# 20171130/Equivariant-NN-Zoo

Hardware: AMD Instinct MI355X
Metric: molecules/s forward+backward, QM9 config_energy batch (higher is better)
Workload: dtype f32

## Files before the change

### equivariant-nn-zoo_amd/csrc/e3k_node.hip

```cpp
#include "e3k_common.h"
#include "e3k_act.h"

namespace e3k {

__global__ __launch_bounds__(256) void act_fwd_kernel(const float* __restrict__ x, int64_t n, int act, float cst,
                                                       float* __restrict__ y) {
  for (int64_t i = (int64_t)blockIdx.x * 256 + threadIdx.x; i < n; i += (int64_t)gridDim.x * 256)
    y[i] = cst * act_f(act, x[i]);
}
__global__ __launch_bounds__(256) void act_bwd_kernel(const float* __restrict__ x, const float* __restrict__ gy,
                                                       int64_t n, int act, float cst, float* __restrict__ gx) {
  for (int64_t i = (int64_t)blockIdx.x * 256 + threadIdx.x; i < n; i += (int64_t)gridDim.x * 256)
    gx[i] = gy[i] * cst * act_df(act, x[i]);
}

__global__ __launch_bounds__(256) void act_bwd2_kernel(const float* __restrict__ x, const float* __restrict__ gy,
                                                        const float* __restrict__ gh, int64_t n, int act, float cst,
                                                        float* __restrict__ g_gy, float* __restrict__ g_x) {
  for (int64_t i = (int64_t)blockIdx.x * 256 + threadIdx.x; i < n; i += (int64_t)gridDim.x * 256) {
    const float xv = x[i], h = gh[i] * cst;
    if (g_gy) g_gy[i] = h * act_df(act, xv);
    if (g_x) g_x[i] = h * gy[i] * act_d2f(act, xv);
  }
}
// ... 246 lines not shown
        case 3: gate_bwd_gated<CF, 3>(s, xr, gr, gr2, gxr, u); break;
        case 5: gate_bwd_gated<CF, 5>(s, xr, gr, gr2, gxr, u); break;
        default: gate_bwd_gated<CF, 7>(s, xr, gr, gr2, gxr, u); break;
      }
    }
  }
}

template <int CF, int DIM>
__device__ __forceinline__ void gate_fwd_gated(const e3k_gate_seg& s, const float* __restrict__ xr, float* __restrict__ yr, int u) {
  float xv[DIM][4];
  const float4 xg4 = ld4(xr + s.gate_off + u);
#pragma unroll
  for (int m = 0; m < DIM; ++m) {
    const float4 a = ld4(xr + s.in_off + m * s.mul + u);
    xv[m][0] = a.x; xv[m][1] = a.y; xv[m][2] = a.z; xv[m][3] = a.w;
  }
  const float sc[4] = {s.cst * act_f(s.act, xg4.x), s.cst * act_f(s.act, xg4.y), s.cst * act_f(s.act, xg4.z),
                       s.cst * act_f(s.act, xg4.w)};
  if (CF) {
#pragma unroll
    for (int m = 0; m < DIM; ++m)
      st4(yr + s.out_off + m * s.mul + u, xv[m][0] * sc[0], xv[m][1] * sc[1], xv[m][2] * sc[2], xv[m][3] * sc[3]);
  } else {
    float v[4 * DIM];
#pragma unroll
    for (int j = 0; j < 4; ++j)
#pragma unroll
      for (int m = 0; m < DIM; ++m) v[j * DIM + m] = xv[m][j] * sc[j];
#pragma unroll
    for (int k = 0; k < DIM; ++k) st4(yr + s.out_off + u * DIM + 4 * k, v[4 * k], v[4 * k + 1], v[4 * k + 2], v[4 * k + 3]);
  }
}

template <int CF>
__global__ __launch_bounds__(256) void gate_fwd4_kernel(const float* __restrict__ x, int64_t rows, int in_dim, int out_dim,
                                                         GateArgs ga, int rb, float* __restrict__ y) {
  const e3k_gate_seg& s = ga.s[blockIdx.y];
  const int q = s.mul >> 2;
  const int64_t row0 = (int64_t)blockIdx.x * rb;
  for (int i = threadIdx.x; i < rb * q; i += 256) {
    const int rr = i / q, u = (i - rr * q) * 4;
    const int64_t r = row0 + rr;
    if (r >= rows) break;
    const float* xr = x + r * in_dim;
    float* yr = y + r * out_dim;
    if (s.kind == 0) {
      const float4 xc = ld4(xr + s.in_off + u);
      st4(yr + s.out_off + u, s.cst * act_f(s.act, xc.x), s.cst * act_f(s.act, xc.y), s.cst * act_f(s.act, xc.z),
          s.cst * act_f(s.act, xc.w));
    } else {
      switch (s.dim) {
        case 1: gate_fwd_gated<CF, 1>(s, xr, yr, u); break;
        case 3: gate_fwd_gated<CF, 3>(s, xr, yr, u); break;
        case 5: gate_fwd_gated<CF, 5>(s, xr, yr, u); break;
        default: gate_fwd_gated<CF, 7>(s, xr, yr, u); break;
      }
    }
  }
}

__global__ __launch_bounds__(256) void gate_bwd2_gy_kernel(const float* __restrict__ x, const float* __restrict__ gh,
                                                            int64_t rows, int in_dim, int out_dim, GateArgs ga,
                                                            float* __restrict__ g_gy) {
  const int c = blockIdx.x * 256 + threadIdx.x;
  if (c >= out_dim) return;
  for (int64_t r = blockIdx.y; r < rows; r += gridDim.y) {
    const int64_t i = r * out_dim + c;
    const float* xr = x + r * in_dim;
    const float* hr = gh + r * in_dim;
    float v = 0.f;
    for (int k = 0; k < ga.n; ++k) {
      const e3k_gate_seg& s = ga.s[k];
      const int rel = c - s.out_off;
      if (rel >= 0 && rel < s.mul * s.dim) {
        if (s.kind == 0) {
          v = hr[s.in_off + rel] * s.cst * act_df(s.act, xr[s.in_off + rel]);
        } else {
          int u, m;
          gate_out_um(s, rel, ga.out_cf, u, m);
          const float gt = xr[s.gate_off + u];
          const int xi = s.in_off + m * s.mul + u;
          v = hr[xi] * (s.cst * act_f(s.act, gt)) + hr[s.gate_off + u] * xr[xi] * (s.cst * act_df(s.act, gt));
        }
        break;
      }
    }
    g_gy[i] = v;
  }
}

__global__ __launch_bounds__(256) void gate_bwd2_x_kernel(const float* __restrict__ x, const float* __restrict__ gy,
                                                           const float* __restrict__ gh, int64_t rows, int in_dim,
                                                           int out_dim, GateArgs ga, float* __restrict__ g_x) {
  const int c = blockIdx.x * 256 + threadIdx.x;
  if (c >= in_dim) return;
  for (int64_t r = blockIdx.y; r < rows; r += gridDim.y) {
    const int64_t i = r * in_dim + c;
    const float* xr = x + r * in_dim;
    const float* hr = gh + r * in_dim;
    const float* gr = gy + r * out_dim;
    float v = 0.f;
    for (int k = 0; k < ga.n; ++k) {
      const e3k_gate_seg& s = ga.s[k];
      if (s.kind == 0) {
        const int rel = c - s.in_off;
        if (rel >= 0 && rel < s.mul) {
          v = hr[c] * gr[s.out_off + rel] * s.cst * act_d2f(s.act, xr[c]);
          break;
        }
      } else {
        const int relg = c - s.gate_off;
        if (relg >= 0 && relg < s.mul) {
          float dgh = 0.f, dgx = 0.f;
          for (int m = 0; m < s.dim; ++m) {
            const float g = gr[gate_out_idx(s, relg, m, ga.out_cf)];
            dgh = fmaf(g, hr[s.in_off + m * s.mul + relg], dgh);
            dgx = fmaf(g, xr[s.in_off + m * s.mul + relg], dgx);
          }
          v = s.cst * (dgh * act_df(s.act, xr[c]) + hr[c] * dgx * act_d2f(s.act, xr[c]));
          break;
        }
        const int rel = c - s.in_off;
        if (rel >= 0 && rel < s.mul * s.dim) {
          const int m = rel / s.mul, u = rel - m * s.mul;
          v = hr[s.gate_off + u] * gr[gate_out_idx(s, u, m, ga.out_cf)] * (s.cst * act_df(s.act, xr[s.gate_off + u]));
          break;
        }
      }
    }
    g_x[i] = v;
  }
}

constexpr int KW_MAXI = 16, KW_MAXV = 32, KW_MAXK = 1 << 22;
struct KwArgs {
  int n, K, V;
  int64_t ld_m, total;
  e3k_kw_instr ins[KW_MAXI];
};

__device__ __forceinline__ const float* kw_locate(const KwArgs& ka, int64_t c, const float* W, int& wout) {
  int j = 0;
  for (int i = 1; i < ka.n; ++i)
    if (c >= ka.ins[i].m_off) j = i;
  const e3k_kw_instr& in = ka.ins[j];
  const int local = (int)(c - in.m_off);
  const int u = local / in.w_out, w = local - u * in.w_out;
  wout = in.w_out;
  return W + in.w_off + (int64_t)u * ka.V * in.w_out + w;
}

constexpr int KW_KT = 64, KW_KT_WIDE = 512;
static inline unsigned kw_tiles(int n_keys, int64_t col_blocks) {
  const int kt = col_blocks >= 1024 ? KW_KT_WIDE : KW_KT;
  return (unsigned)((n_keys + kt - 1) / kt);
}
template <int MODE>
__device__ __forceinline__ void kw_body(const float* __restrict__ a, const float* __restrict__ W, const KwArgs& ka, const int K,
                                        float* __restrict__ M, float* __restrict__ Wout_, int accumulate) {
  const int tile = uniform((K + (int)gridDim.y - 1) / (int)gridDim.y);
  const int t0 = uniform((int)blockIdx.y * tile);
  const int kt = (K - t0 < tile) ? K - t0 : tile;
  if (kt <= 0) return;
  const int V = uniform(ka.V);
  const int64_t c = (int64_t)blockIdx.x * 256 + threadIdx.x;
  if (c >= ka.total) return;
  int wout;
  const float* base = kw_locate(ka, c, W, wout);
  if constexpr (MODE == 0) {
    float wv[KW_MAXV];
#pragma unroll
    for (int v = 0; v < KW_MAXV; ++v) wv[v] = v < V ? base[(int64_t)v * wout] : 0.f;
    for (int t = 0; t < kt; ++t) {
      const float* __restrict__ ar = a + (int64_t)(t0 + t) * V;
      float acc = 0.f;
#pragma unroll
      for (int v = 0; v < KW_MAXV; ++v)
        if (v < V) acc = fmaf(ar[v], wv[v], acc);
      M[(int64_t)(t0 + t) * ka.ld_m + c] = acc;
    }
  } else {
    float gv[KW_MAXV];
#pragma unroll
    for (int v = 0; v < KW_MAXV; ++v) gv[v] = 0.f;
    for (int t = 0; t < kt; ++t) {
      const float* __restrict__ ar = a + (int64_t)(t0 + t) * V;
      const float g = M[(int64_t)(t0 + t) * ka.ld_m + c];
#pragma unroll
      for (int v = 0; v < KW_MAXV; ++v)
        if (v < V) gv[v] = fmaf(ar[v], g, gv[v]);
    }
    float* dst = Wout_ + (base - W);
    if (gridDim.y == 1) {
#pragma unroll
      for (int v = 0; v < KW_MAXV; ++v)
        if (v < V) dst[(int64_t)v * wout] = accumulate ? dst[(int64_t)v * wout] + gv[v] : gv[v];
    } else {
#pragma unroll
      for (int v = 0; v < KW_MAXV; ++v)
        if (v < V) atomicAdd(dst + (int64_t)v * wout, gv[v]);
    }
  }
}

template <int MODE>
__global__ __launch_bounds__(256) void keyed_weights_kernel(const float* __restrict__ a, const float* __restrict__ W,
                                                             KwArgs ka, float* __restrict__ M, float* __restrict__ Wout_,
                                                             int accumulate) {
  kw_body<MODE>(a, W, ka, ka.K, M, Wout_, accumulate);
}

constexpr int KW_MAXL = 8;
struct KwMulti {
  int n, K;
  const KwArgs* ka[KW_MAXL];
  const float* W[KW_MAXL];
  float* M[KW_MAXL];
  float* gW[KW_MAXL];
  int acc[KW_MAXL];
  int64_t ws_off[KW_MAXL];
};
template <int MODE>
__global__ __launch_bounds__(256) void keyed_weights_multi_kernel(const float* __restrict__ a, KwMulti m) {
  const int z = blockIdx.z;
  if (MODE == 1 && !m.gW[z]) return;
  kw_body<MODE>(a, m.W[z], *m.ka[z], m.K, m.M[z], m.gW[z], m.acc[z]);
}

constexpr int KWA_COLS = 256, KWA_KT = 16, KWA_RANGE = 128;
constexpr int KWA_WLD = KWA_COLS + 4;
__device__ __forceinline__ void kw_bwd_a_body(const float* __restrict__ gM, const float* __restrict__ W, const KwArgs& ka_,
                                              const int K, float* __restrict__ ws, float (*gs)[KWA_COLS], float (*wsm)[KWA_WLD]) {
  struct { int K, V; int64_t ld_m, total; } ka{K, ka_.V, ka_.ld_m, ka_.total};
  const int t_id = threadIdx.x;
  const int64_t c = (int64_t)blockIdx.x * KWA_COLS + t_id;
  const bool ok = c < ka.total;
  {
    int wout = 1;
    const float* base = ok ? kw_locate(ka_, c, W, wout) : W;
    for (int v = 0; v < ka.V; ++v) wsm[v][t_id] = ok ? base[(int64_t)v * wout] : 0.f;
  }
  float* out = ws + (int64_t)blockIdx.x * ka.K * ka.V;
  const int t_begin = blockIdx.y * KWA_RANGE;
  const int t_end = (t_begin + KWA_RANGE < ka.K) ? t_begin + KWA_RANGE : ka.K;
  for (int t0 = t_begin; t0 < t_end; t0 += KWA_KT) {
    const int kt = (t_end - t0 < KWA_KT) ? t_end - t0 : KWA_KT;
    __syncthreads();
    for (int t = 0; t < kt; ++t) gs[t][t_id] = ok ? gM[(int64_t)(t0 + t) * ka.ld_m + c] : 0.f;
    __syncthreads();
    for (int o = t_id; o < kt * ka.V; o += 256) {
      const int t = o / ka.V, v = o - t * ka.V;
      const float4* g4 = reinterpret_cast<const float4*>(gs[t]);
      const float4* w4 = reinterpret_cast<const float4*>(wsm[v]);
      float acc = 0.f;
#pragma unroll 8
      for (int q = 0; q < KWA_COLS / 4; ++q) {
        const float4 g = g4[q], w = w4[q];
        acc = fmaf(g.x, w.x, acc);
        acc = fmaf(g.y, w.y, acc);
        acc = fmaf(g.z, w.z, acc);
        acc = fmaf(g.w, w.w, acc);
      }
      out[(t0 + t) * ka.V + v] = acc;
    }
  }
}

__global__ __launch_bounds__(256) void keyed_weights_bwd_a_kernel(const float* __restrict__ gM, const float* __restrict__ W,
                                                                   KwArgs ka, float* __restrict__ ws) {
  __shared__ __attribute__((aligned(16))) float gs[KWA_KT][KWA_COLS];
  __shared__ __attribute__((aligned(16))) float wsm[KW_MAXV][KWA_WLD];
  kw_bwd_a_body(gM, W, ka, ka.K, ws, gs, wsm);
}

__global__ __launch_bounds__(256) void keyed_weights_bwd_a_multi_kernel(KwMulti m, float* __restrict__ ws) {
  __shared__ __attribute__((aligned(16))) float gs[KWA_KT][KWA_COLS];
  __shared__ __attribute__((aligned(16))) float wsm[KW_MAXV][KWA_WLD];
  const int z = blockIdx.z;
  const KwArgs& ka = *m.ka[z];
  if ((int64_t)blockIdx.x * KWA_COLS >= ka.total) return;
  kw_bwd_a_body(m.M[z], m.W[z], ka, m.K, ws + m.ws_off[z] * m.K * ka.V, gs, wsm);
}

__global__ __launch_bounds__(256) void keyed_weights_bwd_a_reduce_kernel(const float* __restrict__ ws, int n_rows, int n,
                                                                          float* __restrict__ ga) {
  const int o = blockIdx.x * 4 + (threadIdx.x >> 6), lane = threadIdx.x & 63;
  if (o >= n) return;
  float acc = 0.f;
  for (int r = lane; r < n_rows; r += 64) acc += ws[(int64_t)r * n + o];
  acc = wave_sum(acc);
  if (lane == 0) ga[o] += acc;
}

__device__ __forceinline__ void normact_scale(int act, float eps2, int normalize, float n2, float& s, float& ds_over_n) {
  if (eps2 > 0.f) {
    const bool clamped = n2 < eps2;
    const float n = sqrtf(clamped ? eps2 : n2);
    const float a = act_f(act, n), da = act_df(act, n);
    if (normalize) {
      s = a / n;
      ds_over_n = clamped ? 0.f : (da * n - a) / (n * n * n);
    } else {
      s = a;
      ds_over_n = clamped ? 0.f : da / n;
    }
  } else {
    s = act_f(act, n2);
    ds_over_n = 2.0f * act_df(act, n2);
  }
}

__global__ __launch_bounds__(256) void normact_fwd_kernel(const float* __restrict__ x, int64_t rows, int row_dim,
                                                           BlockArgs ba, int act, float eps2, int normalize,
                                                           float* __restrict__ y) {
  const int64_t total = rows * row_dim;
  for (int64_t i = (int64_t)blockIdx.x * 256 + threadIdx.x; i < total; i += (int64_t)gridDim.x * 256) {
    const int64_t r = i / row_dim;
    const int c = (int)(i - r * row_dim);
    const float* xr = x + r * row_dim;
    float v = 0.f;
    for (int k = 0; k < ba.n; ++k) {
      const e3k_block& b = ba.b[k];
      const int rel = c - b.off;
      if (rel >= 0 && rel < b.mul * b.dim) {
        const int u = rel / b.dim, m = rel - u * b.dim;
        float n2 = 0.f;
        for (int q = 0; q < b.dim; ++q) {
          const float t = xr[b.off + q * b.mul + u];
          n2 = fmaf(t, t, n2);
        }
        float s, d;
        normact_scale(act, eps2, normalize, n2, s, d);
        v = s * xr[b.off + m * b.mul + u];
        break;
      }
    }
    y[i] = v;
  }
}

__device__ __forceinline__ void normact_scale2(int act, float eps2, int normalize, float n2, float& s, float& d, float& d2) {
  if (eps2 > 0.f) {
    const bool clamped = n2 < eps2;
    const float n = sqrtf(clamped ? eps2 : n2);
    const float a = act_f(act, n), a1 = act_df(act, n), a2 = act_d2f(act, n);
    float s1, s2;
    if (normalize) {
      s = a / n;
      s1 = (a1 * n - a) / (n * n);
      s2 = (a2 * n * n - 2.0f * a1 * n + 2.0f * a) / (n * n * n);
    } else {
      s = a;
      s1 = a1;
      s2 = a2;
    }
    d = clamped ? 0.f : s1 / n;
    d2 = clamped ? 0.f : (s2 * n - s1) / (n * n * n);
  } else {
    s = act_f(act, n2);
    d = 2.0f * act_df(act, n2);
    d2 = 4.0f * act_d2f(act, n2);
  }
}

__global__ __launch_bounds__(256) void normact_bwd2_kernel(const float* __restrict__ x, const float* __restrict__ gy,
                                                            const float* __restrict__ h, int64_t rows, int row_dim, BlockArgs ba,
                                                            int act, float eps2, int normalize, float* __restrict__ g_gy,
                                                            float* __restrict__ g_x) {
  const int64_t total = rows * row_dim;
  for (int64_t i = (int64_t)blockIdx.x * 256 + threadIdx.x; i < total; i += (int64_t)gridDim.x * 256) {
    const int64_t r = i / row_dim;
    const int c = (int)(i - r * row_dim);
    const float* xr = x + r * row_dim;
    const float* gr = gy + r * row_dim;
    const float* hr = h + r * row_dim;
    bool covered = false;
    for (int k = 0; k < ba.n; ++k) {
      const e3k_block& b = ba.b[k];
      const int rel = c - b.off;
      if (rel >= 0 && rel < b.mul * b.dim) {
        covered = true;
        const int m = rel / b.mul, u = rel - m * b.mul;
        float n2 = 0.f, gx_ = 0.f, hx = 0.f, hg = 0.f;
        for (int q = 0; q < b.dim; ++q) {
          const float t = xr[b.off + q * b.mul + u], g = gr[b.off + u * b.dim + q], hh = hr[b.off + q * b.mul + u];
          n2 = fmaf(t, t, n2);
          gx_ = fmaf(g, t, gx_);
          hx = fmaf(hh, t, hx);
          hg = fmaf(hh, g, hg);
        }
        float s, d, d2;
        normact_scale2(act, eps2, normalize, n2, s, d, d2);
        const float xm = xr[c], hm = hr[c], gm = gr[b.off + u * b.dim + m];
        if (g_gy) g_gy[r * row_dim + b.off + u * b.dim + m] = fmaf(s, hm, d * hx * xm);
        if (g_x) g_x[i] = d * xm * hg + d2 * xm * hx * gx_ + d * (hm * gx_ + hx * gm);
        break;
      }
    }
    if (!covered) {
      if (g_gy) g_gy[i] = 0.f;
      if (g_x) g_x[i] = 0.f;
    }
// ... 759 lines not shown
```

### equivariant-nn-zoo_amd/csrc/e3k_rtable.hip

```cpp
#include "e3k_common.h"
#include "e3k_rtable_bwd.h"

namespace e3k {


constexpr int RT_CHUNK = 1024;
__global__ __launch_bounds__(256) void rtable_bins_rank_kernel(const float* __restrict__ r, const int64_t* __restrict__ key, int64_t E,
                                                               float h_inv, int32_t K, int32_t KT, int32_t* __restrict__ bin,
                                                               float* __restrict__ coef, int32_t* __restrict__ lrank,
                                                               int32_t* __restrict__ chunk_hist, int32_t* __restrict__ bad) {
  extern __shared__ int32_t hist_all[];
  const int lane = threadIdx.x & 63, wv = threadIdx.x >> 6;
  int32_t* hist = hist_all + wv * (KT + 1);
  const int64_t chunk = blockIdx.x;
  for (int b = threadIdx.x; b < 4 * (KT + 1); b += 256) hist_all[b] = 0;
  __syncthreads();
  constexpr int PER_WAVE = RT_CHUNK / 4 / 64;
  const int64_t base = chunk * RT_CHUNK + (int64_t)wv * (RT_CHUNK / 4);
  int my_bin[PER_WAVE], my_rank[PER_WAVE];
#pragma unroll
  for (int it = 0; it < PER_WAVE; ++it) {
    const int64_t e = base + it * 64 + lane;
    const bool live = e < E;
    int i = 1;
    if (live) {
      const float raw = r[e] * h_inv;
      float x = raw < 0.f ? 0.f : (raw > (float)K ? (float)K : raw);
      i = (int)x;
      i = i < 1 ? 1 : (i > K - 2 ? K - 2 : i);
      const float t = x - (float)i;
      const float tm1 = t - 1.f, tm2 = t - 2.f, tp1 = t + 1.f;
      float4 c;
      c.x = -t * tm1 * tm2 * (1.f / 6.f);
      c.y = tp1 * tm1 * tm2 * 0.5f;
      c.z = -tp1 * t * tm2 * 0.5f;
      c.w = tp1 * t * tm1 * (1.f / 6.f);
      if (key) {
        const int64_t kk = key[e];
        const int nk = (KT + 1) / (K + 1);
        const bool in_range = kk >= 0 && kk < nk;
        i += in_range ? (int)kk * (K + 1) : 0;
        if (!in_range && bad) atomicOr(bad, 8);
      }
      bin[e] = i;
      *reinterpret_cast<float4*>(coef + 4 * e) = c;
    }
    unsigned long long todo = __ballot(live);
    int rank = 0;
    while (todo) {
      const int leader = __ffsll((long long)todo) - 1;
      const int b = __shfl(i, leader, 64);
      const unsigned long long same = __ballot(live && i == b) & todo;
      const int seen = hist[b];
      if (live && i == b) rank = seen + __popcll(same & ((1ull << lane) - 1ull));
      if (lane == leader) hist[b] = seen + __popcll(same);
      todo &= ~same;
    }
    my_bin[it] = live ? i : -1;
    my_rank[it] = rank;
  }
  __syncthreads();
#pragma unroll
  for (int it = 0; it < PER_WAVE; ++it) {
    if (my_bin[it] < 0) continue;
    int before = 0;
    for (int w = 0; w < wv; ++w) before += hist_all[w * (KT + 1) + my_bin[it]];
    lrank[base + it * 64 + lane] = my_rank[it] + before;
  }
  for (int b = threadIdx.x; b <= KT; b += 256)
    chunk_hist[chunk * (KT + 1) + b] = hist_all[b] + hist_all[(KT + 1) + b] + hist_all[2 * (KT + 1) + b] + hist_all[3 * (KT + 1) + b];
}

__global__ __launch_bounds__(1024) void rtable_bins_scan_kernel(int32_t* __restrict__ chunk_hist, int32_t n_chunks, int32_t K,
                                                                int32_t* __restrict__ ptr, int32_t* __restrict__ seg) {
  __shared__ int32_t wave_tot[2][16];
  __shared__ int32_t carry[2];
  const int t = threadIdx.x, lane = t & 63, w = t >> 6;
  if (t < 2) carry[t] = 0;
  __syncthreads();
  for (int base = 0; base <= K; base += 1024) {
    const int b = base + t;
    int32_t cnt = 0;
    if (b <= K) {
      for (int c = 0; c < n_chunks; ++c) {
        const int32_t v = chunk_hist[(int64_t)c * (K + 1) + b];
        chunk_hist[(int64_t)c * (K + 1) + b] = cnt;
        cnt += v;
      }
    }
    const int32_t sg = (cnt + RT_SEG - 1) / RT_SEG;
    int32_t x = cnt, y = sg;
#pragma unroll
    for (int off = 1; off < 64; off <<= 1) {
      const int32_t xx = __shfl_up(x, off, 64), yy = __shfl_up(y, off, 64);
      if (lane >= off) x += xx, y += yy;
    }
    if (lane == 63) wave_tot[0][w] = x, wave_tot[1][w] = y;
    __syncthreads();
    int32_t bx = carry[0], by = carry[1];
    for (int k = 0; k < w; ++k) bx += wave_tot[0][k], by += wave_tot[1][k];
    if (b <= K) {
      ptr[b] = bx + x - cnt;
      seg[b] = by + y - sg;
      if (b == K) ptr[K + 1] = bx + x, seg[K + 1] = by + y;
    }
    __syncthreads();
    if (t == 1023) carry[0] = bx + x, carry[1] = by + y;
    __syncthreads();
  }
}

__global__ __launch_bounds__(256) void rtable_bins_place_kernel(const int32_t* __restrict__ bin, const int32_t* __restrict__ lrank,
                                                                const int32_t* __restrict__ chunk_off, const int32_t* __restrict__ ptr,
                                                                int64_t E, int32_t K, int32_t* __restrict__ perm) {
  const int64_t e = (int64_t)blockIdx.x * 256 + threadIdx.x;
  if (e >= E) return;
  const int b = bin[e];
  perm[ptr[b] + chunk_off[(e / RT_CHUNK) * (K + 1) + b] + lrank[e]] = (int32_t)e;
}

__global__ __launch_bounds__(256) void rtable_interp_fwd_kernel(const float* __restrict__ T, const int32_t* __restrict__ perm,
                                                                const int32_t* __restrict__ bin, const float* __restrict__ coef,
                                                                int64_t E, int32_t W, float* __restrict__ w,
                                                                const float* __restrict__ T2, float* __restrict__ w2) {
  const int64_t p = (int64_t)blockIdx.x * 4 + (threadIdx.x >> 6);
  if (p >= E) return;
  const int lane = threadIdx.x & 63;
  const int e = uniform(perm[p]);
  const int i = uniform(bin[e]);
  const float* __restrict__ cp = coef + 4 * (int64_t)e;
  const float c0 = __uint_as_float(uniform((int)__float_as_uint(cp[0]))), c1 = __uint_as_float(uniform((int)__float_as_uint(cp[1])));
  const float c2 = __uint_as_float(uniform((int)__float_as_uint(cp[2]))), c3 = __uint_as_float(uniform((int)__float_as_uint(cp[3])));
  const float4* __restrict__ a = reinterpret_cast<const float4*>(T + (int64_t)(i - 1) * W);
  const float4* __restrict__ b = reinterpret_cast<const float4*>(T + (int64_t)i * W);
  const float4* __restrict__ c = reinterpret_cast<const float4*>(T + (int64_t)(i + 1) * W);
  const float4* __restrict__ d = reinterpret_cast<const float4*>(T + (int64_t)(i + 2) * W);
  float4* __restrict__ o = reinterpret_cast<float4*>(w + (int64_t)e * W);
  for (int q = lane; q < (W >> 2); q += 64) {
    const float4 va = a[q], vb = b[q], vc = c[q], vd = d[q];
    float4 v;
    v.x = fmaf(c3, vd.x, fmaf(c2, vc.x, fmaf(c1, vb.x, c0 * va.x)));
    v.y = fmaf(c3, vd.y, fmaf(c2, vc.y, fmaf(c1, vb.y, c0 * va.y)));
    v.z = fmaf(c3, vd.z, fmaf(c2, vc.z, fmaf(c1, vb.z, c0 * va.z)));
    v.w = fmaf(c3, vd.w, fmaf(c2, vc.w, fmaf(c1, vb.w, c0 * va.w)));
    nt_store4(o + q, v);
  }
  if (T2) {
    const int64_t d2 = T2 - T;
    float4* __restrict__ o2 = reinterpret_cast<float4*>(w2 + (int64_t)e * W);
    for (int q = lane; q < (W >> 2); q += 64) {
      const float4 va = reinterpret_cast<const float4*>(reinterpret_cast<const float*>(a) + d2)[q];
      const float4 vb = reinterpret_cast<const float4*>(reinterpret_cast<const float*>(b) + d2)[q];
      const float4 vc = reinterpret_cast<const float4*>(reinterpret_cast<const float*>(c) + d2)[q];
      const float4 vd = reinterpret_cast<const float4*>(reinterpret_cast<const float*>(d) + d2)[q];
      float4 v;
      v.x = fmaf(c3, vd.x, fmaf(c2, vc.x, fmaf(c1, vb.x, c0 * va.x)));
      v.y = fmaf(c3, vd.y, fmaf(c2, vc.y, fmaf(c1, vb.y, c0 * va.y)));
      v.z = fmaf(c3, vd.z, fmaf(c2, vc.z, fmaf(c1, vb.z, c0 * va.z)));
      v.w = fmaf(c3, vd.w, fmaf(c2, vc.w, fmaf(c1, vb.w, c0 * va.w)));
      nt_store4(o2 + q, v);
    }
  }
}

__global__ __launch_bounds__(256) void rtable_bwd_partial_kernel(const float* __restrict__ gw, const float* __restrict__ coef,
                                                                 const float* __restrict__ scale,
                                                                 const int32_t* __restrict__ ptr, const int32_t* __restrict__ seg,
                                                                 const int32_t* __restrict__ perm, int32_t K, int32_t W,
                                                                 int32_t n_chunks, int64_t n_seg_cap, float* __restrict__ P) {
  rtable_bwd_partial_body<8>(gw, coef, scale, ptr, seg, perm, K, W, n_chunks, n_seg_cap, P, (int64_t)blockIdx.x);
}

__global__ __launch_bounds__(256) void rtable_bwd_combine_kernel(const float* __restrict__ P, const int32_t* __restrict__ seg,
                                                                 int32_t K, int32_t W, int32_t accumulate, float* __restrict__ gT) {
  const int64_t q = (int64_t)blockIdx.x * 256 + threadIdx.x;
  const int w4 = W >> 2;
  if (q >= (int64_t)(K + 1) * w4) return;
  const int j = (int)(q / w4), col = (int)(q - (int64_t)j * w4) * 4;
  float4 acc = make_float4(0.f, 0.f, 0.f, 0.f);
  float4* out = reinterpret_cast<float4*>(gT + (int64_t)j * W + col);
  if (accumulate) acc = *out;
#pragma unroll
  for (int k = 0; k < 4; ++k) {
    const int b = j + 1 - k;
    if (b < 1 || b > K - 2) continue;
    const int s0 = seg[b], s1 = seg[b + 1];
    for (int s = s0; s < s1; ++s) {
      const float4 v = *reinterpret_cast<const float4*>(P + ((int64_t)s * 4 + k) * W + col);
      acc.x += v.x; acc.y += v.y; acc.z += v.z; acc.w += v.w;
    }
  }
  *out = acc;
}

typedef _Float16 f16x2 __attribute__((ext_vector_type(2)));
constexpr float PK_S2 = 1024.f, PK_S3 = 65536.f;

__global__ __launch_bounds__(256) void rtable_pack_kernel(const float* __restrict__ T, int32_t K, int32_t W, uint32_t* __restrict__ P) {
  const int64_t q = (int64_t)blockIdx.x * 256 + threadIdx.x;
  if (q >= (int64_t)(K + 1) * W) return;
  const int i = (int)(q / W), col = (int)(q - (int64_t)i * W);
  uint32_t* row = P + 3 * (int64_t)i * W;
  if (i < 1 || i > K - 2) {
    row[2 * col] = row[2 * col + 1] = row[2 * W + col] = 0u;
    return;
  }
  const double a = T[q - W], b = T[q], c = T[q + W], d = T[q + 2 * (int64_t)W];
  const double c1 = -a / 3.0 - b / 2.0 + c - d / 6.0, c2 = a / 2.0 - b + c / 2.0, c3 = -a / 6.0 + b / 2.0 - c / 2.0 + d / 6.0;
  const double e2 = c2 + 1.5 * c3;
  f16x2 h;
  h.x = (_Float16)(float)(e2 * (double)PK_S2);
  h.y = (_Float16)(float)(c3 * (double)PK_S3);
  const double r2 = e2 - (double)(float)h.x / (double)PK_S2, r3 = c3 - (double)(float)h.y / (double)PK_S3;
  const float d0 = (float)(b + c1 / 2.0 + c2 / 4.0 + c3 / 8.0 + r2 / 8.0), d1 = (float)(c1 + c2 + 0.75 * c3 + 3.0 * r3 / 16.0);
  row[2 * col] = __float_as_uint(d0);
  row[2 * col + 1] = __float_as_uint(d1);
  row[2 * W + col] = __builtin_bit_cast(uint32_t, h);
}

struct PackMulti {
  const float* T[16];
  uint32_t* P[16];
  int32_t W[16];
};
__global__ __launch_bounds__(256) void rtable_pack_multi_kernel(PackMulti a, int32_t K) {
  const int tb = blockIdx.y;
  const int32_t W = a.W[tb];
  const int64_t q = (int64_t)blockIdx.x * 256 + threadIdx.x;
  if (q >= (int64_t)(K + 1) * W) return;
  const float* __restrict__ T = a.T[tb];
  const int i = (int)(q / W), col = (int)(q - (int64_t)i * W);
  uint32_t* row = a.P[tb] + 3 * (int64_t)i * W;
  if (i < 1 || i > K - 2) {
    row[2 * col] = row[2 * col + 1] = row[2 * W + col] = 0u;
    return;
  }
  const double ta = T[q - W], b = T[q], c = T[q + W], d = T[q + 2 * (int64_t)W];
  const double c1 = -ta / 3.0 - b / 2.0 + c - d / 6.0, c2 = ta / 2.0 - b + c / 2.0, c3 = -ta / 6.0 + b / 2.0 - c / 2.0 + d / 6.0;
  const double e2 = c2 + 1.5 * c3;
  f16x2 h;
  h.x = (_Float16)(float)(e2 * (double)PK_S2);
  h.y = (_Float16)(float)(c3 * (double)PK_S3);
  const double r2 = e2 - (double)(float)h.x / (double)PK_S2, r3 = c3 - (double)(float)h.y / (double)PK_S3;
  const float d0 = (float)(b + c1 / 2.0 + c2 / 4.0 + c3 / 8.0 + r2 / 8.0), d1 = (float)(c1 + c2 + 0.75 * c3 + 3.0 * r3 / 16.0);
  row[2 * col] = __float_as_uint(d0);
  row[2 * col + 1] = __float_as_uint(d1);
  row[2 * W + col] = __builtin_bit_cast(uint32_t, h);
}

__device__ __forceinline__ float packed_eval(float s, float s2, float s3, float d0, float d1, uint32_t pk) {
  const f16x2 h = __builtin_bit_cast(f16x2, pk);
  return fmaf(s, fmaf(s2, fmaf(s3, (float)h.y, (float)h.x), d1), d0);
}

__global__ __launch_bounds__(256) void rtable_interp_packed_kernel(const uint32_t* __restrict__ P, const int32_t* __restrict__ perm,
                                                                   const int32_t* __restrict__ bin, const float* __restrict__ coef,
                                                                   int64_t E, int32_t W, float* __restrict__ w) {
  const int64_t p = (int64_t)blockIdx.x * 4 + (threadIdx.x >> 6);
  if (p >= E) return;
  const int lane = threadIdx.x & 63;
  const int e = uniform(perm[p]);
  const int i = uniform(bin[e]);
  const float* __restrict__ cp = coef + 4 * (int64_t)e;
  const float c0 = __uint_as_float(uniform((int)__float_as_uint(cp[0]))), c2 = __uint_as_float(uniform((int)__float_as_uint(cp[2])));
  const float c3 = __uint_as_float(uniform((int)__float_as_uint(cp[3])));
  const float s = fmaf(2.f, c3, c2 - c0) - 0.5f, s2 = s * (1.f / PK_S2), s3 = s * (PK_S2 / PK_S3);
  const uint32_t* __restrict__ row = P + 3 * (int64_t)i * W;
  float* __restrict__ o = w + (int64_t)e * W;
  for (int q = lane; q < W; q += 64) o[q] = packed_eval(s, s2, s3, __uint_as_float(row[2 * q]), __uint_as_float(row[2 * q + 1]), row[2 * W + q]);
}

struct GuardArgs {
  const float* T[16];
  float* state[16];
  float* scratch[16];
  int32_t W[16];
  int32_t rows;
  float floor_rel, c4, col_weight, pack_weight;
};

__device__ __forceinline__ void atomic_max_pos(float* p, float v) {
  atomicMax(reinterpret_cast<unsigned int*>(p), __float_as_uint(v));
}

constexpr int RT_GUARD_PARTS = 8;
__global__ __launch_bounds__(256) void rtable_guard_kernel(GuardArgs a) {
  __shared__ float s_col[4][64], s_d4[4][64];
  const int tb = blockIdx.y;
  const int W = a.W[tb];
  const int n_chunks = (W + 63) / 64;
  if ((int)blockIdx.x >= n_chunks) return;
  const float* __restrict__ T = a.T[tb];
  const int lane = threadIdx.x & 63, q = threadIdx.x >> 6;
  const int col = blockIdx.x * 64 + lane;
  const int rows = a.rows;
  const int n_d4 = rows - 4;
  const int per = (n_d4 + 4 * RT_GUARD_PARTS - 1) / (4 * RT_GUARD_PARTS);
  const int rq = blockIdx.z * 4 + q;
  const int lo = rq * per < n_d4 ? rq * per : n_d4, hi = (lo + per < n_d4) ? lo + per : n_d4;
  float cmax = 0.f, dmax = 0.f;
  bool bad = false;
  if (col < W && lo < hi) {
    float v0 = T[(int64_t)lo * W + col], v1 = T[(int64_t)(lo + 1) * W + col], v2 = T[(int64_t)(lo + 2) * W + col],
          v3 = T[(int64_t)(lo + 3) * W + col];
    cmax = fmaxf(fmaxf(fabsf(v0), fabsf(v1)), fmaxf(fabsf(v2), fabsf(v3)));
    bad = !(fabsf(v0) < INFINITY) || !(fabsf(v1) < INFINITY) || !(fabsf(v2) < INFINITY) || !(fabsf(v3) < INFINITY);
    for (int i = lo; i < hi; ++i) {
      const float v4 = T[(int64_t)(i + 4) * W + col];
      bad = bad || !(fabsf(v4) < INFINITY);
      cmax = fmaxf(cmax, fabsf(v4));
      const float d4 = (v4 + v0) - 4.f * (v3 + v1) + 6.f * v2;
      const float d2 = (v1 + v3) - 2.f * v2, d3 = (v3 - v0) - 3.f * (v2 - v1);
      dmax = fmaxf(dmax, a.c4 * fabsf(d4) + a.pack_weight * (1.f / 2048.f) * (fabsf(d2) * (1.f / 16.f) + fabsf(d3) * (1.f / 192.f)));
      v0 = v1; v1 = v2; v2 = v3; v3 = v4;
    }
  }
  s_col[q][lane] = bad ? INFINITY : cmax;
  s_d4[q][lane] = bad ? INFINITY : dmax;
  __syncthreads();
  if (q == 0 && col < W) {
    float* __restrict__ mine = a.scratch[tb] + (int64_t)blockIdx.z * 2 * W;
    mine[col] = fmaxf(fmaxf(s_col[0][lane], s_col[1][lane]), fmaxf(s_col[2][lane], s_col[3][lane]));
    mine[W + col] = fmaxf(fmaxf(s_d4[0][lane], s_d4[1][lane]), fmaxf(s_d4[2][lane], s_d4[3][lane]));
  }
}

__global__ __launch_bounds__(256) void rtable_guard_reduce_kernel(GuardArgs a) {
  __shared__ float s_red[4], s_red2[4];
  const int tb = blockIdx.x;
  const int W = a.W[tb];
  const float* __restrict__ scratch = a.scratch[tb];
  const int lane = threadIdx.x & 63, q = threadIdx.x >> 6;
  float g = 0.f;
  auto fold = [&](int c, float& cm, float& dm) {
    cm = 0.f, dm = 0.f;
#pragma unroll
    for (int z = 0; z < RT_GUARD_PARTS; ++z) {
      cm = fmaxf(cm, scratch[(int64_t)z * 2 * W + c]);
      dm = fmaxf(dm, scratch[(int64_t)z * 2 * W + W + c]);
    }
  };
  for (int c = threadIdx.x; c < W; c += 256) {
// ... 186 lines not shown
```

Measured before the change: 94990.

## Batch loads for memory-level parallelism across keyed-weight and rtable kernels

The keyed-weights forward and backward bodies now handle keys in blocks of 4/2/1 and load activation chunks up front. The backward preloads old weight values and gradient rows. The bwd-a kernel prefetches the next gradient tile into registers while the current tile is computed. The rtable rank kernel swaps the serial leader loop for a fixed 64-step readlane/ballot match, and the scan and combine kernels batch their loads. All of this aims to hide memory latency by keeping more loads in flight, at the cost of more registers and possibly lower occupancy.

```diff
diff --git a/equivariant-nn-zoo_amd/csrc/e3k_node.hip b/equivariant-nn-zoo_amd/csrc/e3k_node.hip
--- a/equivariant-nn-zoo_amd/csrc/e3k_node.hip
+++ b/equivariant-nn-zoo_amd/csrc/e3k_node.hip
@@ -422,9 +422,48 @@
 }
 
 constexpr int KW_KT = 64, KW_KT_WIDE = 512;
+constexpr int KW_SB = 4, KW_KB = 8, KW_VC = 4;
 static inline unsigned kw_tiles(int n_keys, int64_t col_blocks) {
   const int kt = col_blocks >= 1024 ? KW_KT_WIDE : KW_KT;
   return (unsigned)((n_keys + kt - 1) / kt);
+}
+template <int NB, class F>
+__device__ __forceinline__ void kw_chunks(const float* __restrict__ ab, const int V, F&& f) {
+#pragma unroll
+  for (int v0 = 0; v0 < KW_MAXV; v0 += KW_VC) {
+    if (v0 + KW_VC <= V) {
+      float x[NB][KW_VC];
+#pragma unroll
+      for (int i = 0; i < NB; ++i)
+#pragma unroll
+        for (int q = 0; q < KW_VC; ++q) x[i][q] = ab[i * V + v0 + q];
+#pragma unroll
+      for (int i = 0; i < NB; ++i)
+#pragma unroll
+        for (int q = 0; q < KW_VC; ++q) f(i, v0 + q, x[i][q]);
+    } else if (v0 < V) {
+#pragma unroll
+      for (int q = 0; q < KW_VC - 1; ++q)
+        if (v0 + q < V) {
+#pragma unroll
+          for (int i = 0; i < NB; ++i) f(i, v0 + q, ab[i * V + v0 + q]);
+        }
+    }
+  }
+}
+template <int NB>
+__device__ __forceinline__ void kw_fwd_keys(const float* __restrict__ ab, const int V, const float (&wv)[KW_MAXV],
+                                            float* __restrict__ Mp, const int64_t ld_m) {
+  float acc[NB];
+#pragma unroll
+  for (int i = 0; i < NB; ++i) acc[i] = 0.f;
+  kw_chunks<NB>(ab, V, [&](int i, int v, float x) { acc[i] = fmaf(x, wv[v], acc[i]); });
+#pragma unroll
+  for (int i = 0; i < NB; ++i) Mp[(int64_t)i * ld_m] = acc[i];
+}
+template <int NB>
+__device__ __forceinline__ void kw_bwd_keys(const float* __restrict__ ab, const int V, const float* g, float (&gv)[KW_MAXV]) {
+  kw_chunks<NB>(ab, V, [&](int i, int v, float x) { gv[v] = fmaf(x, g[i], gv[v]); });
 }
 template <int MODE>
 __device__ __forceinline__ void kw_body(const float* __restrict__ a, const float* __restrict__ W, const KwArgs& ka, const int K,
@@ -442,30 +481,47 @@
     float wv[KW_MAXV];
 #pragma unroll
     for (int v = 0; v < KW_MAXV; ++v) wv[v] = v < V ? base[(int64_t)v * wout] : 0.f;
-    for (int t = 0; t < kt; ++t) {
-      const float* __restrict__ ar = a + (int64_t)(t0 + t) * V;
-      float acc = 0.f;
+    const float* __restrict__ ab = a + (int64_t)t0 * V;
+    float* __restrict__ Mp = M + (int64_t)t0 * ka.ld_m + c;
+    int tb = 0;
+    for (; tb + KW_SB <= kt; tb += KW_SB) kw_fwd_keys<KW_SB>(ab + (int64_t)tb * V, V, wv, Mp + (int64_t)tb * ka.ld_m, ka.ld_m);
+    static_assert(KW_SB == 4, "the rest below: 2, 1 keys");
+    if (kt - tb >= 2) kw_fwd_keys<2>(ab + (int64_t)tb * V, V, wv, Mp + (int64_t)tb * ka.ld_m, ka.ld_m), tb += 2;
+    if (kt - tb >= 1) kw_fwd_keys<1>(ab + (int64_t)tb * V, V, wv, Mp + (int64_t)tb * ka.ld_m, ka.ld_m);
+  } else {
+    float* dst = Wout_ + (base - W);
+    const bool stores = gridDim.y == 1;
+    float old[KW_MAXV];
+#pragma unroll
+    for (int v = 0; v < KW_MAXV; ++v) old[v] = (stores && accumulate && v < V) ? dst[(int64_t)v * wout] : 0.f;
+    float gv[KW_MAXV];
+#pragma unroll
+    for (int v = 0; v < KW_MAXV; ++v) gv[v] = 0.f;
+    const float* __restrict__ gp = M + (int64_t)t0 * ka.ld_m + c;
+    const float* __restrict__ ab = a + (int64_t)t0 * V;
+    for (int tb = 0; tb < kt; tb += KW_KB) {
+      float g[KW_KB];
+#pragma unroll
+      for (int i = 0; i < KW_KB; ++i) g[i] = tb + i < kt ? gp[(int64_t)(tb + i) * ka.ld_m] : 0.f;
+      const float* __restrict__ abk = ab + (int64_t)tb * V;
+      int nb = kt - tb < KW_KB ? kt - tb : KW_KB;
+      static_assert(KW_KB == 8 && KW_SB == 4, "blocks of 4 keys, then 2, 1; g moves down so that every index into it is a constant");
+      for (; nb >= 4; nb -= 4) {
+        kw_bwd_keys<4>(abk, V, g, gv);
+        abk += 4 * V;
+        g[0] = g[4], g[1] = g[5], g[2] = g[6], g[3] = g[7];
+      }
+      if (nb >= 2) {
+        kw_bwd_keys<2>(abk, V, g, gv);
+        abk += 2 * V, nb -= 2;
+        g[0] = g[2];
+      }
+      if (nb >= 1) kw_bwd_keys<1>(abk, V, g, gv);
+    }
+    if (stores) {
 #pragma unroll
       for (int v = 0; v < KW_MAXV; ++v)
-        if (v < V) acc = fmaf(ar[v], wv[v], acc);
-      M[(int64_t)(t0 + t) * ka.ld_m + c] = acc;
-    }
-  } else {
-    float gv[KW_MAXV];
-#pragma unroll
-    for (int v = 0; v < KW_MAXV; ++v) gv[v] = 0.f;
-    for (int t = 0; t < kt; ++t) {
-      const float* __restrict__ ar = a + (int64_t)(t0 + t) * V;
-      const float g = M[(int64_t)(t0 + t) * ka.ld_m + c];
-#pragma unroll
-      for (int v = 0; v < KW_MAXV; ++v)
-        if (v < V) gv[v] = fmaf(ar[v], g, gv[v]);
-    }
-    float* dst = Wout_ + (base - W);
-    if (gridDim.y == 1) {
-#pragma unroll
-      for (int v = 0; v < KW_MAXV; ++v)
-        if (v < V) dst[(int64_t)v * wout] = accumulate ? dst[(int64_t)v * wout] + gv[v] : gv[v];
+        if (v < V) dst[(int64_t)v * wout] = accumulate ? old[v] + gv[v] : gv[v];
     } else {
 #pragma unroll
       for (int v = 0; v < KW_MAXV; ++v)
@@ -506,19 +562,33 @@
   const int t_id = threadIdx.x;
   const int64_t c = (int64_t)blockIdx.x * KWA_COLS + t_id;
   const bool ok = c < ka.total;
+  const int t_begin = blockIdx.y * KWA_RANGE;
+  const int t_end = (t_begin + KWA_RANGE < ka.K) ? t_begin + KWA_RANGE : ka.K;
+  float greg[KWA_KT];
+  auto fetch = [&](int t0) {
+#pragma unroll
+    for (int t = 0; t < KWA_KT; ++t) greg[t] = (ok && t0 + t < t_end) ? gM[(int64_t)(t0 + t) * ka.ld_m + c] : 0.f;
+  };
   {
     int wout = 1;
     const float* base = ok ? kw_locate(ka_, c, W, wout) : W;
-    for (int v = 0; v < ka.V; ++v) wsm[v][t_id] = ok ? base[(int64_t)v * wout] : 0.f;
+    float wreg[KW_MAXV];
+#pragma unroll
+    for (int v = 0; v < KW_MAXV; ++v) wreg[v] = (ok && v < ka.V) ? base[(int64_t)v * wout] : 0.f;
+    fetch(t_begin);
+#pragma unroll
+    for (int v = 0; v < KW_MAXV; ++v)
+      if (v < ka.V) wsm[v][t_id] = wreg[v];
   }
   float* out = ws + (int64_t)blockIdx.x * ka.K * ka.V;
-  const int t_begin = blockIdx.y * KWA_RANGE;
-  const int t_end = (t_begin + KWA_RANGE < ka.K) ? t_begin + KWA_RANGE : ka.K;
   for (int t0 = t_begin; t0 < t_end; t0 += KWA_KT) {
     const int kt = (t_end - t0 < KWA_KT) ? t_end - t0 : KWA_KT;
     __syncthreads();
-    for (int t = 0; t < kt; ++t) gs[t][t_id] = ok ? gM[(int64_t)(t0 + t) * ka.ld_m + c] : 0.f;
+#pragma unroll
+    for (int t = 0; t < KWA_KT; ++t)
+      if (t < kt) gs[t][t_id] = greg[t];
     __syncthreads();
+    if (t0 + KWA_KT < t_end) fetch(t0 + KWA_KT);
     for (int o = t_id; o < kt * ka.V; o += 256) {
       const int t = o / ka.V, v = o - t * ka.V;
       const float4* g4 = reinterpret_cast<const float4*>(gs[t]);
diff --git a/equivariant-nn-zoo_amd/csrc/e3k_rtable.hip b/equivariant-nn-zoo_amd/csrc/e3k_rtable.hip
--- a/equivariant-nn-zoo_amd/csrc/e3k_rtable.hip
+++ b/equivariant-nn-zoo_amd/csrc/e3k_rtable.hip
@@ -45,18 +45,29 @@
       bin[e] = i;
       *reinterpret_cast<float4*>(coef + 4 * e) = c;
     }
-    unsigned long long todo = __ballot(live);
+    my_bin[it] = live ? i : -1;
+  }
+  unsigned long long same[PER_WAVE];
+#pragma unroll
+  for (int it = 0; it < PER_WAVE; ++it) same[it] = 0ull;
+#pragma unroll 8
+  for (int j = 0; j < 64; ++j) {
+#pragma unroll
+    for (int it = 0; it < PER_WAVE; ++it) {
+      const bool eq = my_bin[it] == __builtin_amdgcn_readlane(my_bin[it], j);
+      const unsigned long long m = __ballot(eq);
+      if (eq) same[it] = m;
+    }
+  }
+#pragma unroll
+  for (int it = 0; it < PER_WAVE; ++it) {
     int rank = 0;
-    while (todo) {
-      const int leader = __ffsll((long long)todo) - 1;
-      const int b = __shfl(i, leader, 64);
-      const unsigned long long same = __ballot(live && i == b) & todo;
-      const int seen = hist[b];
-      if (live && i == b) rank = seen + __popcll(same & ((1ull << lane) - 1ull));
-      if (lane == leader) hist[b] = seen + __popcll(same);
-      todo &= ~same;
-    }
-    my_bin[it] = live ? i : -1;
+    if (my_bin[it] >= 0) {
+      const int before = __popcll(same[it] & ((1ull << lane) - 1ull));
+      const int seen = hist[my_bin[it]];
+      rank = seen + before;
+      if (before == 0) hist[my_bin[it]] = seen + __popcll(same[it]);
+    }
     my_rank[it] = rank;
   }
   __syncthreads();
@@ -71,6 +82,7 @@
     chunk_hist[chunk * (KT + 1) + b] = hist_all[b] + hist_all[(KT + 1) + b] + hist_all[2 * (KT + 1) + b] + hist_all[3 * (KT + 1) + b];
 }
 
+constexpr int RT_SCAN_B = 16;
 __global__ __launch_bounds__(1024) void rtable_bins_scan_kernel(int32_t* __restrict__ chunk_hist, int32_t n_chunks, int32_t K,
                                                                 int32_t* __restrict__ ptr, int32_t* __restrict__ seg) {
   __shared__ int32_t wave_tot[2][16];
@@ -82,10 +94,18 @@
     const int b = base + t;
     int32_t cnt = 0;
     if (b <= K) {
-      for (int c = 0; c < n_chunks; ++c) {
-        const int32_t v = chunk_hist[(int64_t)c * (K + 1) + b];
-        chunk_hist[(int64_t)c * (K + 1) + b] = cnt;
-        cnt += v;
+      int32_t* col = chunk_hist + b;
+      const int64_t ld = K + 1;
+      for (int c0 = 0; c0 < n_chunks; c0 += RT_SCAN_B) {
+        int32_t v[RT_SCAN_B];
+#pragma unroll
+        for (int i = 0; i < RT_SCAN_B; ++i) v[i] = c0 + i < n_chunks ? col[(int64_t)(c0 + i) * ld] : 0;
+#pragma unroll
+        for (int i = 0; i < RT_SCAN_B; ++i)
+          if (c0 + i < n_chunks) {
+            col[(int64_t)(c0 + i) * ld] = cnt;
+            cnt += v[i];
+          }
       }
     }
     const int32_t sg = (cnt + RT_SEG - 1) / RT_SEG;
@@ -171,6 +191,7 @@
   rtable_bwd_partial_body<8>(gw, coef, scale, ptr, seg, perm, K, W, n_chunks, n_seg_cap, P, (int64_t)blockIdx.x);
 }
 
+constexpr int RT_COMB_B = 4;
 __global__ __launch_bounds__(256) void rtable_bwd_combine_kernel(const float* __restrict__ P, const int32_t* __restrict__ seg,
                                                                  int32_t K, int32_t W, int32_t accumulate, float* __restrict__ gT) {
   const int64_t q = (int64_t)blockIdx.x * 256 + threadIdx.x;
@@ -179,15 +200,34 @@
   const int j = (int)(q / w4), col = (int)(q - (int64_t)j * w4) * 4;
   float4 acc = make_float4(0.f, 0.f, 0.f, 0.f);
   float4* out = reinterpret_cast<float4*>(gT + (int64_t)j * W + col);
-  if (accumulate) acc = *out;
+  int s0[4], s1[4];
 #pragma unroll
   for (int k = 0; k < 4; ++k) {
     const int b = j + 1 - k;
-    if (b < 1 || b > K - 2) continue;
-    const int s0 = seg[b], s1 = seg[b + 1];
-    for (int s = s0; s < s1; ++s) {
-      const float4 v = *reinterpret_cast<const float4*>(P + ((int64_t)s * 4 + k) * W + col);
-      acc.x += v.x; acc.y += v.y; acc.z += v.z; acc.w += v.w;
+    const bool has = b >= 1 && b <= K - 2;
+    s0[k] = has ? seg[b] : 0;
+    s1[k] = has ? seg[b + 1] : 0;
+  }
+  if (accumulate) acc = *out;
+  const float4 zero = make_float4(0.f, 0.f, 0.f, 0.f);
+  auto row = [&](int s, int k) { return *reinterpret_cast<const float4*>(P + ((int64_t)s * 4 + k) * W + col); };
+  float4 v[4][RT_COMB_B];
+#pragma unroll
+  for (int k = 0; k < 4; ++k)
+#pragma unroll
+    for (int i = 0; i < RT_COMB_B; ++i) v[k][i] = s0[k] + i < s1[k] ? row(s0[k] + i, k) : zero;
+#pragma unroll
+  for (int k = 0; k < 4; ++k) {
+#pragma unroll
+    for (int i = 0; i < RT_COMB_B; ++i)
+      if (s0[k] + i < s1[k]) acc.x += v[k][i].x, acc.y += v[k][i].y, acc.z += v[k][i].z, acc.w += v[k][i].w;
+    for (int s = s0[k] + RT_COMB_B; s < s1[k]; s += RT_COMB_B) {
+      float4 u[RT_COMB_B];
+#pragma unroll
+      for (int i = 0; i < RT_COMB_B; ++i) u[i] = s + i < s1[k] ? row(s + i, k) : zero;
+#pragma unroll
+      for (int i = 0; i < RT_COMB_B; ++i)
+        if (s + i < s1[k]) acc.x += u[i].x, acc.y += u[i].y, acc.z += u[i].z, acc.w += u[i].w;
     }
   }
   *out = acc;
```

Measured after the change: 96490, median of 6. 1.6% higher.
